# xqtr/PySpecSDR

Measured on AMD Instinct MI355X. Metric: IQ MSamples/sec end-to-end (FFT+dB+FM demod), higher is better.
Workload: dtype complex64 IQ / f64 FFT + dB + post-process + FIR + IIR / dB rows stored as f32 / int16 PCM

## Files before the change

### pyspecsdr_amd/csrc/pss_api.cpp

```cpp
#include <hip/hip_runtime.h>

#include <cstdlib>
#include <cstring>
#include <string>
#include <vector>

#include "pss_ctx.h"

static std::string g_create_err;

int pss_fail(pss_ctx *ctx, int code, const std::string &msg)
{
    if (ctx) ctx->err = msg;
    else g_create_err = msg;
    return code;
}

int pss_hip_check(pss_ctx *ctx, hipError_t e, const char *what)
{
    if (e == hipSuccess) return PSS_OK;
    return pss_fail(ctx, PSS_E_HIP, std::string(what) + ": " + hipGetErrorString(e));
}

int pss_ensure_buffer(pss_ctx *ctx, void **buf, size_t *cap, size_t bytes, const char *what)
{
    if (bytes <= *cap) return PSS_OK;
    if (*buf) {
        hipStreamSynchronize(ctx->stream);
        if (ctx->stream2) hipStreamSynchronize(ctx->stream2);
        hipFree(*buf);
        *buf = nullptr;
        *cap = 0;
    }
    hipError_t e = hipMalloc(buf, bytes);
    if (e != hipSuccess) return pss_fail(ctx, PSS_E_NOMEM, std::string(what) + " hipMalloc: " + hipGetErrorString(e));
    *cap = bytes;
    return PSS_OK;
}

int pss_ensure_scratch(pss_ctx *ctx, size_t bytes)
{
    return pss_ensure_buffer(ctx, &ctx->scratch, &ctx->scratch_bytes, bytes, "scratch");
}

void pss_time_begin(pss_ctx *ctx)
{
    if (ctx->timing && ctx->tdepth++ == 0 && ctx->tfilter.empty()) hipEventRecord(ctx->ev0, ctx->stream);
}
void pss_kernel_begin(pss_ctx *ctx, const char *name)
{
    if (!ctx->timing) return;
    ctx->kskip = !ctx->tfilter.empty() && ctx->tfilter != name;
    if (ctx->kskip) return;
    if (ctx->kused == (int)ctx->krecs.size()) {
        pss_ctx::KRec r{name, nullptr, nullptr};
        hipEventCreate(&r.e0);
        hipEventCreate(&r.e1);
        ctx->krecs.push_back(r);
    }
    ctx->krecs[ctx->kused].name = name;
    hipEventRecord(ctx->krecs[ctx->kused].e0, PSS_STREAM(ctx));
}
void pss_kernel_end(pss_ctx *ctx)
{
    if (!ctx->timing || ctx->kskip) return;
    hipEventRecord(ctx->krecs[ctx->kused].e1, PSS_STREAM(ctx));
    ctx->kused++;
}
void pss_time_end(pss_ctx *ctx)
{
    if (ctx->timing && --ctx->tdepth == 0) {
        if (ctx->tfilter.empty()) hipEventRecord(ctx->ev1, ctx->stream);
        ctx->last_ms = 0.0f;
    }
}

extern "C" int pss_device_count(void)
{
    int n = 0;
    if (hipGetDeviceCount(&n) != hipSuccess) return 0;
    return n;
}

extern "C" int pss_create(int device, pss_ctx **out)
{
    if (!out) return PSS_E_ARG;
    *out = nullptr;
    int n = 0;
    hipError_t e = hipGetDeviceCount(&n);
    if (e != hipSuccess || n <= 0)
        return pss_fail(nullptr, PSS_E_HIP, std::string("no HIP device available (libpss has no CPU fallback): ") +
                                                (e != hipSuccess ? hipGetErrorString(e) : "device count is 0"));
    if (device < 0 || device >= n) return pss_fail(nullptr, PSS_E_ARG, "device index out of range");
    int prev = -1;
    hipGetDevice(&prev);
    e = hipSetDevice(device);
    if (e != hipSuccess) return pss_fail(nullptr, PSS_E_HIP, std::string("hipSetDevice: ") + hipGetErrorString(e));
    struct Restore {
        int prev, dev;
        ~Restore() { if (prev >= 0 && prev != dev) hipSetDevice(prev); }
    } restore{prev, device};
    pss_ctx *ctx = new pss_ctx();
    ctx->device = device;
    { int cus = 0; if (hipDeviceGetAttribute(&cus, hipDeviceAttributeMultiprocessorCount, device) == hipSuccess) ctx->n_cus = cus; }
    { const char *e = getenv("PSS_NO_FUSED"); ctx->no_fused = e && e[0] == '1'; }
    e = hipStreamCreateWithFlags(&ctx->stream, hipStreamNonBlocking);
    if (e == hipSuccess) ctx->own_stream = true;
    if (e == hipSuccess) e = hipEventCreate(&ctx->ev0);
    if (e == hipSuccess) e = hipEventCreate(&ctx->ev1);
    if (e == hipSuccess) e = hipStreamCreateWithFlags(&ctx->stream2, hipStreamNonBlocking);
    if (e == hipSuccess) e = hipEventCreateWithFlags(&ctx->ev_fork, hipEventDisableTiming);
    if (e == hipSuccess) e = hipEventCreateWithFlags(&ctx->ev_join, hipEventDisableTiming);
    if (e != hipSuccess) {
        const std::string msg = std::string("context stream / event creation: ") + hipGetErrorString(e);
        if (ctx->ev0) hipEventDestroy(ctx->ev0);
        if (ctx->ev1) hipEventDestroy(ctx->ev1);
        if (ctx->ev_fork) hipEventDestroy(ctx->ev_fork);
        if (ctx->ev_join) hipEventDestroy(ctx->ev_join);
        if (ctx->stream2) hipStreamDestroy(ctx->stream2);
        if (ctx->own_stream) hipStreamDestroy(ctx->stream);
        delete ctx;
        return pss_fail(nullptr, PSS_E_HIP, msg);
    }
    *out = ctx;
    return PSS_OK;
}

extern "C" void pss_destroy(pss_ctx *ctx)
{
    if (!ctx) return;
    PssDevGuard guard(ctx->device);
    hipStreamSynchronize(ctx->stream);
    if (ctx->comm) pss_comm_free(ctx);
    for (auto &kv : ctx->tw) hipFree(kv.second);
    for (auto &kv : ctx->tw_pf) hipFree(kv.second);
    for (auto &kv : ctx->win) hipFree(kv.second);
    for (auto &kv : ctx->bs) { hipFree(kv.second.d_chirp); hipFree(kv.second.d_B); hipFree(kv.second.d_win); }
    for (auto &kv : ctx->plans) {
        hipFree(kv.second.d_leaf_off); hipFree(kv.second.d_leaf_len); hipFree(kv.second.d_node_l);
        hipFree(kv.second.d_node_r); hipFree(kv.second.d_level_start); hipFree(kv.second.d_roots);
    }
    for (auto &kv : ctx->nfm) if (kv.second.d_rev) hipFree(kv.second.d_rev);
    if (ctx->scratch) hipFree(ctx->scratch);
    if (ctx->scratch_fft) hipFree(ctx->scratch_fft);
    if (ctx->scratch_hil) hipFree(ctx->scratch_hil);
    if (ctx->scratch_iqc) hipFree(ctx->scratch_iqc);
    if (ctx->d_hann) hipFree(ctx->d_hann);
    if (ctx->d_hann_short) hipFree(ctx->d_hann_short);
    if (ctx->st_up) hipStreamDestroy(ctx->st_up);
    if (ctx->st_dn) hipStreamDestroy(ctx->st_dn);
    for (auto &e : ctx->st_ev) if (e) hipEventDestroy(e);
    for (auto &b : ctx->st_buf) if (b) hipFree(b);
    if (ctx->scratch_scan) hipFree(ctx->scratch_scan);
    if (ctx->scratch_pk) hipFree(ctx->scratch_pk);
    if (ctx->scratch_win) hipFree(ctx->scratch_win);
    if (ctx->scratch_db64) hipFree(ctx->scratch_db64);
    if (ctx->scratch_post) hipFree(ctx->scratch_post);
    if (ctx->prog) hipFree(ctx->prog);
    if (ctx->stage) hipFree(ctx->stage);
    hipEventDestroy(ctx->ev0);
    hipEventDestroy(ctx->ev1);
    hipStreamSynchronize(ctx->stream2);
    hipStreamDestroy(ctx->stream2);
    hipEventDestroy(ctx->ev_fork);
    hipEventDestroy(ctx->ev_join);
    if (ctx->ev_in) hipEventDestroy(ctx->ev_in);
    if (ctx->ev_out) hipEventDestroy(ctx->ev_out);
    for (auto &k : ctx->krecs) { hipEventDestroy(k.e0); hipEventDestroy(k.e1); }
    if (ctx->own_stream) hipStreamDestroy(ctx->stream);
    delete ctx;
}

extern "C" int pss_set_stream(pss_ctx *ctx, void *hip_stream)
{
    if (!ctx) return PSS_E_ARG;
    PSS_GUARD(ctx);
    hipStreamSynchronize(ctx->stream);
    if (ctx->own_stream) hipStreamDestroy(ctx->stream);
    ctx->stream = reinterpret_cast<hipStream_t>(hip_stream);
    ctx->own_stream = false;
    return PSS_OK;
}

extern "C" int pss_order_after(pss_ctx *ctx, void *hip_stream)
{
    if (!ctx) return PSS_E_ARG;
    PSS_GUARD(ctx);
    hipStream_t s = reinterpret_cast<hipStream_t>(hip_stream);
    if (s == ctx->stream) return PSS_OK;
    if (!ctx->ev_in) PSS_HIP(ctx, hipEventCreateWithFlags(&ctx->ev_in, hipEventDisableTiming));
    PSS_HIP(ctx, hipEventRecord(ctx->ev_in, s));
    PSS_HIP(ctx, hipStreamWaitEvent(ctx->stream, ctx->ev_in, 0));
    return PSS_OK;
}

extern "C" int pss_order_before(pss_ctx *ctx, void *hip_stream)
{
    if (!ctx) return PSS_E_ARG;
    PSS_GUARD(ctx);
    hipStream_t s = reinterpret_cast<hipStream_t>(hip_stream);
    if (s == ctx->stream) return PSS_OK;
    if (!ctx->ev_out) PSS_HIP(ctx, hipEventCreateWithFlags(&ctx->ev_out, hipEventDisableTiming));
    PSS_HIP(ctx, hipEventRecord(ctx->ev_out, ctx->stream));
    PSS_HIP(ctx, hipStreamWaitEvent(s, ctx->ev_out, 0));
    return PSS_OK;
}

extern "C" void *pss_get_stream(pss_ctx *ctx) { return ctx ? reinterpret_cast<void *>(ctx->stream) : nullptr; }

extern "C" int pss_set_option(pss_ctx *ctx, const char *key, int value)
{
    if (!ctx || !key) return PSS_E_ARG;
    if (!strcmp(key, "nfm_fused")) { ctx->no_fused = (value == 0); return PSS_OK; }
    if (!strcmp(key, "wfm_fused")) { ctx->no_wfm_fused = (value == 0); return PSS_OK; }
    if (!strcmp(key, "small_batch")) { ctx->no_small_batch = (value == 0); return PSS_OK; }
    if (!strcmp(key, "small_batch_max")) { ctx->small_batch_max = value; return PSS_OK; }
    if (!strcmp(key, "wfm_small_batch_max")) { ctx->wfm_small_batch_max = value; return PSS_OK; }
    if (!strcmp(key, "fuse_post")) { ctx->fuse_post = value != 0; return PSS_OK; }
    if (!strcmp(key, "ssb_rfft")) { ctx->ssb_rfft = value != 0; return PSS_OK; }
    if (!strcmp(key, "ssb_hilbert")) { ctx->ssb_hilbert = value != 0; return PSS_OK; }
    if (!strcmp(key, "hilbert_exact")) { ctx->hilbert_exact = value != 0; return PSS_OK; }
    if (!strcmp(key, "scan_exact")) { ctx->scan_exact = value != 0; return PSS_OK; }
    if (!strcmp(key, "db_exact")) { ctx->db_exact = value != 0; return PSS_OK; }
    if (!strcmp(key, "f64_plain")) { ctx->f64_plain = value != 0; return PSS_OK; }
    if (!strcmp(key, "wfm_corr_copy")) { ctx->wfm_corr_copy = value != 0; return PSS_OK; }
    return pss_fail(ctx, PSS_E_ARG, std::string("unknown option: ") + key);
}

extern "C" int pss_sync(pss_ctx *ctx)
{
    if (!ctx) return PSS_E_ARG;
    PSS_GUARD(ctx);
    return pss_hip_check(ctx, hipStreamSynchronize(ctx->stream), "hipStreamSynchronize");
}

extern "C" const char *pss_last_error(pss_ctx *ctx) { return ctx ? ctx->err.c_str() : g_create_err.c_str(); }

extern "C" int pss_enable_timing(pss_ctx *ctx, int on)
{
    if (!ctx) return PSS_E_ARG;
    PSS_GUARD(ctx);
    ctx->timing = on != 0;
    ctx->tdepth = 0;
    ctx->kused = 0;
    ctx->last_ms = -1.0f;
    return PSS_OK;
}

extern "C" int pss_timing_filter(pss_ctx *ctx, const char *kernel)
{
    if (!ctx) return PSS_E_ARG;
    PSS_GUARD(ctx);
    ctx->tfilter = kernel ? kernel : "";
    ctx->kused = 0;
    ctx->last_ms = -1.0f;
    return PSS_OK;
}

extern "C" float pss_last_kernel_ms(pss_ctx *ctx)
{
    if (!ctx || !ctx->timing || ctx->last_ms < 0.0f || !ctx->tfilter.empty()) return -1.0f;
    PSS_GUARD(ctx);
    if (hipEventSynchronize(ctx->ev1) != hipSuccess) return -1.0f;
    float ms = -1.0f;
    if (hipEventElapsedTime(&ms, ctx->ev0, ctx->ev1) != hipSuccess) return -1.0f;
    return ms;
}

extern "C" int pss_kernel_times(pss_ctx *ctx, char *buf, int buf_len)
{
    if (!ctx || !buf || buf_len < 1) return PSS_E_ARG;
    PSS_GUARD(ctx);
    std::string out;
    if (ctx->timing && ctx->last_ms >= 0.0f) {
        if (ctx->tfilter.empty()) hipEventSynchronize(ctx->ev1);
        else hipStreamSynchronize(ctx->stream);
        for (int i = 0; i < ctx->kused; i++) {
            float ms = 0.0f;
            if (hipEventElapsedTime(&ms, ctx->krecs[i].e0, ctx->krecs[i].e1) != hipSuccess) continue;
            out += ctx->krecs[i].name;
            out += "=" + std::to_string(ms) + ";";
        }
    }
    ctx->kused = 0;
    if ((int)out.size() + 1 > buf_len) return pss_fail(ctx, PSS_E_ARG, "buffer too small");
    memcpy(buf, out.c_str(), out.size() + 1);
    return PSS_OK;
}

namespace {
size_t up256(size_t x) { return (x + 255) & ~(size_t)255; }
}

extern "C" int pss_h_compute_fft(pss_ctx *ctx, const float *h_iq, int n, double *h_db)
{
    if (!ctx) return PSS_E_ARG;
    PSS_GUARD(ctx);
    if (!h_iq || !h_db || n < 1) return pss_fail(ctx, PSS_E_ARG, "bad arguments");
    const size_t o_db = up256(sizeof(float) * 2 * n);
    int r = pss_ensure_buffer(ctx, &ctx->stage, &ctx->stage_bytes, o_db + up256(sizeof(float) * n), "staging");
    if (r) return r;
    char *base = reinterpret_cast<char *>(ctx->stage);
    PSS_HIP(ctx, hipMemcpyAsync(base, h_iq, sizeof(float) * 2 * n, hipMemcpyHostToDevice, ctx->stream));
    r = pss_spectrum_db(ctx, reinterpret_cast<const float *>(base), 1, n, reinterpret_cast<float *>(base + o_db));
    if (r) return r;
    std::vector<float> tmp(n);
    PSS_HIP(ctx, hipMemcpyAsync(tmp.data(), base + o_db, sizeof(float) * n, hipMemcpyDeviceToHost, ctx->stream));
    PSS_HIP(ctx, hipStreamSynchronize(ctx->stream));
    for (int i = 0; i < n; i++) h_db[i] = (double)tmp[i];
    return PSS_OK;
}
// ... 521 lines not shown
```

### pyspecsdr_amd/csrc/pss_ctx.h

```cpp
#pragma once
#include <hip/hip_runtime.h>

#include <array>
#include <functional>
#include <map>
#include <string>
#include <vector>

#include "../../include/pss.h"

struct PssNfmFilt {
    double taps[65];
    double sos[24];
    double zi[8];
    double *d_rev = nullptr;
};

struct PssWfmFilt {
    double lp[18], pilot[30], lmr[30];
    double alpha;
};

struct PssPairwisePlan {
    int n_leaves = 0, n_nodes = 0, n_levels = 0, n_roots = 0;
    int wave_tree = 0;
    int *d_leaf_off = nullptr, *d_leaf_len = nullptr, *d_node_l = nullptr, *d_node_r = nullptr, *d_level_start = nullptr;
    int *d_roots = nullptr;
};

struct pss_ctx {
    int device = 0;
    hipStream_t stream = nullptr;
    bool own_stream = false;
    hipStream_t stream2 = nullptr;
    hipStream_t cur = nullptr;
    hipEvent_t ev_fork = nullptr, ev_join = nullptr;
    hipEvent_t ev_in = nullptr, ev_out = nullptr;
    int n_cus = 0;
    bool iq_c128 = false;
    int fuse_post = 1;
    double target_rate = 22050.0;
    bool wfm_correct = false;
    const float *wfm_scal = nullptr;
    bool wfm_corr_copy = false;
    float *power_out = nullptr;
    bool fork_after_fwd = false;
    bool did_fork = false;
    bool defer_bwd = false;
    std::function<int()> pending_bwd;
    std::string err;
    std::map<int, double2 *> tw;
    std::map<int, double *> win;
    std::map<int, double2 *> tw_pf;
    struct Bluestein { double2 *d_chirp; double2 *d_B; double *d_win; int M; };
    std::map<int, Bluestein> bs;
    std::map<double, PssNfmFilt> nfm;
    std::map<double, std::array<double, 65>> ssb;
    std::map<double, PssWfmFilt> wfm;
    std::map<int, PssPairwisePlan> plans;
    void *scratch = nullptr;
    size_t scratch_bytes = 0;
    void *scratch_iqc = nullptr;
    void *scratch_scan = nullptr;
    size_t scratch_scan_bytes = 0;
    void *scratch_pk = nullptr;
    size_t scratch_pk_bytes = 0;
    void *prog = nullptr;
    unsigned prog_epoch = 0;
    void *scratch_post = nullptr;
    size_t scratch_post_bytes = 0;
    void *scratch_db64 = nullptr;
    size_t scratch_db64_bytes = 0;
    void *scratch_win = nullptr;
    size_t scratch_win_bytes = 0;
    float *d_hann = nullptr;
    float hann_sum = 0.0f;
    hipStream_t st_up = nullptr, st_dn = nullptr;
    hipEvent_t st_ev[6] = {nullptr, nullptr, nullptr, nullptr, nullptr, nullptr};
    void *st_buf[18] = {};
    size_t st_cap[18] = {};
    float *d_hann_short = nullptr;
    float hann_short_sum = 0.0f;
    int hann_short_n = 0;
    size_t scratch_iqc_bytes = 0;
    void *scratch_fft = nullptr;
    size_t scratch_fft_bytes = 0;
    void *scratch_hil = nullptr;
    size_t scratch_hil_bytes = 0;
    void *stage = nullptr;
    size_t stage_bytes = 0;
    bool no_wfm_fused = false;
    long small_batch_max = 8192;
    long wfm_small_batch_max = 6000;
    bool hilbert_exact = false;
    bool ssb_rfft = true;
    bool ssb_hilbert = true;
    bool db_exact = false;
    bool f64_plain = false;
    bool scan_exact = true;
    bool no_small_batch = false;
    bool no_fused = false;
    void *comm = nullptr;
    int comm_rank = 0, comm_n = 1;
    bool timing = false;
    std::string tfilter;
    bool kskip = false;
    int tdepth = 0;
    hipEvent_t ev0 = nullptr, ev1 = nullptr;
    float last_ms = -1.0f;
    struct KRec { const char *name; hipEvent_t e0, e1; };
    std::vector<KRec> krecs;
    int kused = 0;
};

struct PssDevGuard {
    int prev = -1;
    bool switched = false;
    explicit PssDevGuard(int dev)
    {
        if (hipGetDevice(&prev) == hipSuccess && prev != dev) switched = hipSetDevice(dev) == hipSuccess;
    }
    ~PssDevGuard()
    {
        if (switched) hipSetDevice(prev);
    }
    PssDevGuard(const PssDevGuard &) = delete;
    PssDevGuard &operator=(const PssDevGuard &) = delete;
};
#define PSS_GUARD(ctx) PssDevGuard _pss_dev_guard((ctx)->device)

template <class T>
struct PssScoped {
    T &ref;
    T keep;
    PssScoped(T &r, T v) : ref(r), keep(r) { r = v; }
    ~PssScoped() { ref = keep; }
    PssScoped(const PssScoped &) = delete;
    PssScoped &operator=(const PssScoped &) = delete;
};
using PssFlagScope = PssScoped<bool>;
using PssStreamScope = PssScoped<hipStream_t>;

int pss_fail(pss_ctx *ctx, int code, const std::string &msg);
int pss_hip_check(pss_ctx *ctx, hipError_t e, const char *what);
int pss_ensure_scratch(pss_ctx *ctx, size_t bytes);
int pss_ensure_buffer(pss_ctx *ctx, void **buf, size_t *cap, size_t bytes, const char *what);
void pss_time_begin(pss_ctx *ctx);
void pss_time_end(pss_ctx *ctx);
void pss_kernel_begin(pss_ctx *ctx, const char *name);
void pss_kernel_end(pss_ctx *ctx);

#define PSS_STREAM(ctx) ((ctx)->cur ? (ctx)->cur : (ctx)->stream)

#define PSS_HIP(ctx, call)                                         \
    do {                                                           \
        int _r = pss_hip_check((ctx), (call), #call);              \
        if (_r) return _r;                                         \
    } while (0)

bool pss_hilbert_supported(int n);
int pss_hilbert_rows(pss_ctx *ctx, const double *d_x, long n_rows, int n, double *d_out, int out_mode, unsigned long long *d_maxbits,
                     int16_t *d_pcm);
int pss_fft_tables(pss_ctx *ctx, int n, const double2 **tw, const double **win);
bool pss_post_sel_serves(int n_fft, bool f64);
bool pss_spec_post_serves(const pss_ctx *ctx, int n_fft);
int pss_spec_post_chain(pss_ctx *ctx, const float *d_iq, long n_frames, int n_fft, float *d_db32, double *d_db64, double *d_lo, double *d_hi, int n_halo,
                        int window, int display, int disp_h, int disp_w, int8_t *d_a, int8_t *d_b, double *d_vals);
int pss_chain_vals_f32(pss_ctx *ctx, const float *d_db, long n_frames, int n_fft, float *d_lo, float *d_hi, int n_halo, int window, int display,
                       int disp_h, int disp_w, int8_t *d_a, int8_t *d_b, double *d_vals);
int pss_chain_vals_f64(pss_ctx *ctx, const double *d_db, long n_frames, int n_fft, double *d_lo, double *d_hi, int n_halo, int window, int display,
                       int disp_h, int disp_w, int8_t *d_a, int8_t *d_b, double *d_vals);
bool pss_ssb_fused_supported(int n);
double pss_np_tan(double x);
double pss_np_exp(double x);
int pss_ssb_hilbert_fused(pss_ctx *ctx, const float *d_iq, long n_rows, int n, const double *taps65, double *d_audio, int16_t *d_pcm);
```

### pyspecsdr_amd/csrc/pss_fft.hip

```cpp
#include <hip/hip_runtime.h>

#include <cmath>
#include <vector>

#include "pss_ctx.h"
#include "pss_fft_r16.h"
#include "pss_fft_xl.h"
#include "pss_post.h"
#include "pss_spec_post.h"
#include "pss_hilbert.h"
#include "pss_hilbert_pf.h"

namespace {

constexpr int TPB = 256;

inline int spec_flags(const pss_ctx *ctx) { return (ctx->scan_exact ? pss_r16::FLAG_SCAN_EXACT : 0) | (ctx->db_exact ? pss_r16::FLAG_DB_EXACT : 0); }
constexpr int LOG_NSUB_MAX = 12;
constexpr int STAGE_MAX_N = 16384;
constexpr int PT = 1024;

__device__ __forceinline__ double2 cmul(double2 a, double2 b)
{
    return make_double2(a.x * b.x - a.y * b.y, a.x * b.y + a.y * b.x);
// ... 1491 lines not shown
        pss_time_end(ctx);
        return pss_hip_check(ctx, hipGetLastError(), "k_disp_vals_win launch");
    }
    int r = pss_ensure_buffer(ctx, &ctx->scratch_win, &ctx->scratch_win_bytes, (size_t)n_frames * 2 * sizeof(double), "window extremes");
    if (r) { pss_time_end(ctx); return r; }
    double *wlo = reinterpret_cast<double *>(ctx->scratch_win), *whi = wlo + n_frames;
    pss_kernel_begin(ctx, "k_slide_extremes");
    hipLaunchKernelGGL(pss_post::k_slide_extremes<T>, dim3((unsigned)((n_frames + 255) / 256 < 4096 ? (n_frames + 255) / 256 : 4096)),
                       dim3(256), 0, PSS_STREAM(ctx), d_lo, d_hi, n_frames, n_halo, window, wlo, whi);
    pss_kernel_end(ctx);
    const long cells = n_frames * disp_w;
    pss_kernel_begin(ctx, "k_disp_rows");
    const dim3 dgrid((unsigned)((cells + 255) / 256 < 16384 ? (cells + 255) / 256 : 16384));
    if (d_thr)
        hipLaunchKernelGGL((pss_post::k_disp_rows<T, MODE, true>), dgrid, dim3(256), 0, PSS_STREAM(ctx), d_post, wlo, whi, n_frames, len,
                           disp_w, disp_h, d_a, d_b, d_thr);
    else
        hipLaunchKernelGGL((pss_post::k_disp_rows<T, MODE>), dgrid, dim3(256), 0, PSS_STREAM(ctx), d_post, wlo, whi, n_frames, len, disp_w,
                           disp_h, d_a, d_b, (const T *)nullptr);
    pss_kernel_end(ctx);
    pss_time_end(ctx);
    return pss_hip_check(ctx, hipGetLastError(), "k_disp_rows launch");
}

}

extern "C" int pss_spectrum_db_post(pss_ctx *ctx, const float *d_iq, long n_frames, int n_fft, float *d_db, float *d_post,
                                    float *d_row_lo, float *d_row_hi)
{
    if (!ctx) return PSS_E_ARG;
    PSS_GUARD(ctx);
    if (n_frames < 0 || (n_frames > 0 && (!d_iq || !d_db || !d_post))) return pss_fail(ctx, PSS_E_ARG, "pss_spectrum_db_post: null buffer");
    if ((d_row_lo == nullptr) != (d_row_hi == nullptr)) return pss_fail(ctx, PSS_E_ARG, "row extremes: pass both arrays or neither");
    if (n_frames == 0) return PSS_OK;
    int r = pss_spectrum_db(ctx, d_iq, n_frames, n_fft, d_db);
    if (!r) r = spectrum_post(ctx, d_db, n_frames, n_fft, d_post, d_row_lo, d_row_hi);
    return r;
}

extern "C" int pss_spectrum_post(pss_ctx *ctx, const float *d_db, long n_frames, int n_fft, float *d_post)
{
    if (!ctx) return PSS_E_ARG;
    PSS_GUARD(ctx);
    return spectrum_post(ctx, d_db, n_frames, n_fft, d_post, nullptr, nullptr);
}

extern "C" int pss_spectrum_post_extremes(pss_ctx *ctx, const float *d_db, long n_frames, int n_fft, float *d_post, float *d_row_lo,
                                          float *d_row_hi)
{
    if (!ctx) return PSS_E_ARG;
    PSS_GUARD(ctx);
    if (n_frames > 0 && (!d_row_lo || !d_row_hi)) return pss_fail(ctx, PSS_E_ARG, "null row-extremes array");
    return spectrum_post(ctx, d_db, n_frames, n_fft, d_post, d_row_lo, d_row_hi);
}

extern "C" int pss_row_extremes(pss_ctx *ctx, const float *d_rows, long n_rows, int len, float *d_row_lo, float *d_row_hi)
{
    if (!ctx) return PSS_E_ARG;
    PSS_GUARD(ctx);
    return row_extremes<float>(ctx, d_rows, n_rows, len, d_row_lo, d_row_hi);
}
extern "C" int pss_row_extremes_f64(pss_ctx *ctx, const double *d_rows, long n_rows, int len, double *d_row_lo, double *d_row_hi)
{
    if (!ctx) return PSS_E_ARG;
    PSS_GUARD(ctx);
    return row_extremes<double>(ctx, d_rows, n_rows, len, d_row_lo, d_row_hi);
}

extern "C" int pss_spectrum_post_f64(pss_ctx *ctx, const double *d_db, long n_frames, int n_fft, double *d_post, double *d_row_lo, double *d_row_hi)
{
    if (!ctx) return PSS_E_ARG;
    PSS_GUARD(ctx);
    if (n_frames < 0 || n_fft < 5 || (n_frames > 0 && (!d_db || !d_post))) return pss_fail(ctx, PSS_E_ARG, "pss_spectrum_post_f64: bad argument");
    if ((d_row_lo == nullptr) != (d_row_hi == nullptr)) return pss_fail(ctx, PSS_E_ARG, "pss_spectrum_post_f64: row_lo and row_hi go together");
    if (n_frames == 0) return PSS_OK;
    if (!ctx->f64_plain && n_fft >= 8 && post_sel_serves(n_fft, true)) {
        pss_time_begin(ctx);
        const int rq = post_sel_any<double>(ctx, d_db, n_frames, n_fft, d_post, d_row_lo, d_row_hi, nullptr, nullptr, 0);
        pss_time_end(ctx);
        return rq;
    }
    pss_time_begin(ctx);
    pss_kernel_begin(ctx, "k_post_f64");
    hipLaunchKernelGGL(k_post_f64, dim3((unsigned)(n_frames < 2048 ? n_frames : 2048)), dim3(256), 0, PSS_STREAM(ctx), d_db, d_post, n_fft, n_frames);
    pss_kernel_end(ctx);
    int r = pss_hip_check(ctx, hipGetLastError(), "k_post_f64 launch");
    if (!r && d_row_lo) r = row_extremes<double>(ctx, d_post, n_frames, n_fft - 4, d_row_lo, d_row_hi);
    pss_time_end(ctx);
    return r;
}

extern "C" int pss_spectrum_post_thresholds(pss_ctx *ctx, const float *d_db, long n_frames, int n_fft, float *d_row_thr, float *d_row_lo,
                                            float *d_row_hi)
{
    if (!ctx) return PSS_E_ARG;
    PSS_GUARD(ctx);
    if (n_frames > 0 && (!d_row_thr || !d_row_lo || !d_row_hi)) return pss_fail(ctx, PSS_E_ARG, "pss_spectrum_post_thresholds: null buffer");
    return spectrum_post(ctx, d_db, n_frames, n_fft, nullptr, d_row_lo, d_row_hi, d_row_thr);
}
extern "C" int pss_waterfall_rows_db(pss_ctx *ctx, const float *d_db, long n_frames, int n_fft, const float *d_row_thr, const float *d_row_lo,
                                     const float *d_row_hi, int n_halo, int window, int disp_w, int8_t *d_glyph, int8_t *d_colour)
{
    if (!ctx) return PSS_E_ARG;
    PSS_GUARD(ctx);
    if (n_frames > 0 && !d_row_thr) return pss_fail(ctx, PSS_E_ARG, "pss_waterfall_rows_db: null thresholds");
    return display_rows<float, 0>(ctx, d_db, n_frames, n_fft - 4, d_row_lo, d_row_hi, n_halo, window, 1, disp_w, d_glyph, d_colour, d_row_thr);
}
extern "C" int pss_persistence_rows_db(pss_ctx *ctx, const float *d_db, long n_frames, int n_fft, const float *d_row_thr,
                                       const float *d_row_lo, const float *d_row_hi, int n_halo, int window, int disp_h, int disp_w, int8_t *d_y)
{
    if (!ctx) return PSS_E_ARG;
    PSS_GUARD(ctx);
    if (n_frames > 0 && !d_row_thr) return pss_fail(ctx, PSS_E_ARG, "pss_persistence_rows_db: null thresholds");
    return display_rows<float, 1>(ctx, d_db, n_frames, n_fft - 4, d_row_lo, d_row_hi, n_halo, window, disp_h, disp_w, d_y, nullptr, d_row_thr);
}

bool pss_post_sel_serves(int n_fft, bool f64) { return n_fft >= 8 && post_sel_serves(n_fft, f64); }
template <class TR>
static int chain_vals(pss_ctx *ctx, const TR *d_db, long n_frames, int n_fft, TR *d_lo, TR *d_hi, int n_halo, int window, int display, int disp_h,
                      int disp_w, int8_t *d_a, int8_t *d_b, double *d_vals)
{
    if (n_frames == 0) return PSS_OK;
    pss_time_begin(ctx);
    int r = post_sel_any<TR>(ctx, d_db, n_frames, n_fft, (TR *)nullptr, d_lo + n_halo, d_hi + n_halo, (TR *)nullptr, d_vals, disp_w);
    if (!r) r = display ? display_rows<TR, 1>(ctx, (const TR *)nullptr, n_frames, n_fft - 4, d_lo, d_hi, n_halo, window, disp_h, disp_w, d_a, nullptr, (const TR *)nullptr, d_vals)
                        : display_rows<TR, 0>(ctx, (const TR *)nullptr, n_frames, n_fft - 4, d_lo, d_hi, n_halo, window, 1, disp_w, d_a, d_b, (const TR *)nullptr, d_vals);
    pss_time_end(ctx);
    return r;
}
int pss_chain_vals_f32(pss_ctx *ctx, const float *d_db, long n_frames, int n_fft, float *d_lo, float *d_hi, int n_halo, int window, int display,
                       int disp_h, int disp_w, int8_t *d_a, int8_t *d_b, double *d_vals)
{
    return chain_vals<float>(ctx, d_db, n_frames, n_fft, d_lo, d_hi, n_halo, window, display, disp_h, disp_w, d_a, d_b, d_vals);
}
int pss_chain_vals_f64(pss_ctx *ctx, const double *d_db, long n_frames, int n_fft, double *d_lo, double *d_hi, int n_halo, int window, int display,
                       int disp_h, int disp_w, int8_t *d_a, int8_t *d_b, double *d_vals)
{
    return chain_vals<double>(ctx, d_db, n_frames, n_fft, d_lo, d_hi, n_halo, window, display, disp_h, disp_w, d_a, d_b, d_vals);
}

bool pss_spec_post_serves(const pss_ctx *ctx, int n_fft) { return n_fft == 1024 && !ctx->f64_plain; }
int pss_spec_post_chain(pss_ctx *ctx, const float *d_iq, long n_frames, int n_fft, float *d_db32, double *d_db64, double *d_lo, double *d_hi,
                        int n_halo, int window, int display, int disp_h, int disp_w, int8_t *d_a, int8_t *d_b, double *d_vals)
{
    if (!pss_spec_post_serves(ctx, n_fft) || (!d_db32 && !d_db64)) return pss_fail(ctx, PSS_E_ARG, "fused transform + post-process: 1024-point frames, a row buffer");
    if (n_frames == 0) return PSS_OK;
    const double2 *tw;
    const double *win;
    int r = pss_fft_tables(ctx, n_fft, &tw, &win);
    if (r) return r;
    using C = pss_r16::Cfg<2>;
    auto kern = d_db32 ? (d_db64 ? pss_sp::k_spectrum_post<true, true> : pss_sp::k_spectrum_post<true, false>) : pss_sp::k_spectrum_post<false, true>;
    const size_t lds = (size_t)C::FPW * C::EX * sizeof(double2) + (size_t)C::TW2 * sizeof(double2);
    const long cap = 256L * 2 * 2;
    if (lds > 64 * 1024) PSS_HIP(ctx, hipFuncSetAttribute(reinterpret_cast<const void *>(kern), hipFuncAttributeMaxDynamicSharedMemorySize, (int)lds));
    const long groups = (n_frames + C::FPW - 1) / C::FPW;
    pss_time_begin(ctx);
    pss_kernel_begin(ctx, "k_spectrum_post");
    hipLaunchKernelGGL(kern, dim3((unsigned)(groups < cap ? groups : cap)), dim3(256), lds, PSS_STREAM(ctx), reinterpret_cast<const float2 *>(d_iq), d_db32,
                       d_db64, tw, win, n_frames, d_lo + n_halo, d_hi + n_halo, d_vals, disp_w);
    pss_kernel_end(ctx);
    r = pss_hip_check(ctx, hipGetLastError(), "k_spectrum_post launch");
    if (!r) r = display ? display_rows<double, 1>(ctx, (const double *)nullptr, n_frames, n_fft - 4, d_lo, d_hi, n_halo, window, disp_h, disp_w, d_a, nullptr, (const double *)nullptr, d_vals)
                        : display_rows<double, 0>(ctx, (const double *)nullptr, n_frames, n_fft - 4, d_lo, d_hi, n_halo, window, 1, disp_w, d_a, d_b, (const double *)nullptr, d_vals);
    pss_time_end(ctx);
    return r;
}

extern "C" int pss_waterfall_rows(pss_ctx *ctx, const float *d_post, long n_frames, int len, const float *d_row_lo,
                                  const float *d_row_hi, int n_halo, int window, int disp_w, int8_t *d_glyph, int8_t *d_colour)
{
    if (!ctx) return PSS_E_ARG;
    PSS_GUARD(ctx);
    return display_rows<float, 0>(ctx, d_post, n_frames, len, d_row_lo, d_row_hi, n_halo, window, 1, disp_w, d_glyph, d_colour);
}
extern "C" int pss_waterfall_rows_f64(pss_ctx *ctx, const double *d_post, long n_frames, int len, const double *d_row_lo,
                                      const double *d_row_hi, int n_halo, int window, int disp_w, int8_t *d_glyph, int8_t *d_colour)
{
    if (!ctx) return PSS_E_ARG;
    PSS_GUARD(ctx);
    return display_rows<double, 0>(ctx, d_post, n_frames, len, d_row_lo, d_row_hi, n_halo, window, 1, disp_w, d_glyph, d_colour);
}
extern "C" int pss_persistence_rows(pss_ctx *ctx, const float *d_post, long n_frames, int len, const float *d_row_lo,
                                    const float *d_row_hi, int n_halo, int window, int disp_h, int disp_w, int8_t *d_y)
{
    if (!ctx) return PSS_E_ARG;
    PSS_GUARD(ctx);
    return display_rows<float, 1>(ctx, d_post, n_frames, len, d_row_lo, d_row_hi, n_halo, window, disp_h, disp_w, d_y, nullptr);
}
extern "C" int pss_persistence_rows_f64(pss_ctx *ctx, const double *d_post, long n_frames, int len, const double *d_row_lo,
                                        const double *d_row_hi, int n_halo, int window, int disp_h, int disp_w, int8_t *d_y)
{
    if (!ctx) return PSS_E_ARG;
    PSS_GUARD(ctx);
    return display_rows<double, 1>(ctx, d_post, n_frames, len, d_row_lo, d_row_hi, n_halo, window, disp_h, disp_w, d_y, nullptr);
}

extern "C" int pss_waterfall_cells(pss_ctx *ctx, const float *d_rows, int n_rows, int len, int disp_h, int disp_w,
                                   int8_t *d_glyph, int8_t *d_colour)
{
    if (!ctx) return PSS_E_ARG;
    PSS_GUARD(ctx);
    if (!d_rows || !d_glyph || !d_colour || n_rows < 1 || len < 2 || disp_h < 1 || disp_w < 1)
        return pss_fail(ctx, PSS_E_ARG, "bad waterfall arguments");
    pss_kernel_begin(ctx, "k_cells");
    hipLaunchKernelGGL((k_cells<float, 0>), dim3(1), dim3(1024), 0, PSS_STREAM(ctx), d_rows, n_rows, len, disp_h, disp_w,
                       d_glyph, d_colour, 0, n_rows);
    pss_kernel_end(ctx);
    return pss_hip_check(ctx, hipGetLastError(), "k_cells launch");
}

extern "C" int pss_persistence_cells(pss_ctx *ctx, const float *d_rows, int n_rows, int len, int disp_h, int disp_w,
                                     int8_t *d_colour)
{
    if (!ctx) return PSS_E_ARG;
    PSS_GUARD(ctx);
    if (!d_rows || !d_colour || n_rows < 1 || len < 2 || disp_h < 1 || disp_w < 1)
        return pss_fail(ctx, PSS_E_ARG, "bad persistence arguments");
    pss_kernel_begin(ctx, "k_cells");
    hipLaunchKernelGGL((k_cells<float, 1>), dim3(1), dim3(1024), 0, PSS_STREAM(ctx), d_rows, n_rows, len, disp_h, disp_w,
                       (int8_t *)nullptr, d_colour, 0, n_rows);
    pss_kernel_end(ctx);
    return pss_hip_check(ctx, hipGetLastError(), "k_cells launch");
}

template <class T>
static int launch_spectrogram(pss_ctx *ctx, const T *d_rows, long n_rows, int len, int disp_h, int disp_w, int8_t *d_glyph,
                              int8_t *d_colour, double *d_range)
{
    if (!ctx) return PSS_E_ARG;
    PSS_GUARD(ctx);
    if (!d_rows || !d_glyph || !d_colour || n_rows < 0 || len < 2 || disp_h < 1 || disp_w < 1)
        return pss_fail(ctx, PSS_E_ARG, "bad spectrogram arguments");
    if (n_rows == 0) return PSS_OK;
    pss_kernel_begin(ctx, "k_spectrogram");
    hipLaunchKernelGGL(k_spectrogram<T>, dim3((unsigned)(n_rows < 4096 ? n_rows : 4096)), dim3(len <= 4096 ? 256 : 1024), 0,
                       PSS_STREAM(ctx), d_rows, n_rows, len, disp_h, disp_w, d_glyph, d_colour, d_range);
    pss_kernel_end(ctx);
    return pss_hip_check(ctx, hipGetLastError(), "k_spectrogram launch");
}

extern "C" int pss_spectrogram_cells(pss_ctx *ctx, const float *d_rows, long n_rows, int len, int disp_h, int disp_w,
                                     int8_t *d_glyph, int8_t *d_colour, double *d_range)
{
    return launch_spectrogram<float>(ctx, d_rows, n_rows, len, disp_h, disp_w, d_glyph, d_colour, d_range);
}

extern "C" int pss_spectrogram_cells_f64(pss_ctx *ctx, const double *d_rows, long n_rows, int len, int disp_h, int disp_w,
                                         int8_t *d_glyph, int8_t *d_colour, double *d_range)
{
    return launch_spectrogram<double>(ctx, d_rows, n_rows, len, disp_h, disp_w, d_glyph, d_colour, d_range);
}

__global__ __launch_bounds__(256) void k_vector(const float2 *__restrict__ iq, int n, int max_h, int max_w, int8_t *__restrict__ grid)
{
    const int cx = max_w / 2, cy = max_h / 2, scale = (max_w < max_h ? max_w : max_h) / 4;
    for (int k = blockIdx.x * blockDim.x + threadIdx.x; k < n; k += gridDim.x * blockDim.x) {
        const float2 v = iq[k];
        const float fx = __fadd_rn((float)cx, __fmul_rn(v.x, (float)scale)), fy = __fsub_rn((float)cy, __fmul_rn(v.y, (float)scale));
        if (!isfinite(fx) || !isfinite(fy)) continue;
        const int x = (int)fx, y = (int)fy;
        if (x >= 0 && x < max_w && y >= 0 && y < max_h) grid[y * max_w + x] = 1;
    }
}

extern "C" int pss_vector_cells(pss_ctx *ctx, const float *d_iq, int n, int max_h, int max_w, int8_t *d_grid)
{
    if (!ctx) return PSS_E_ARG;
    PSS_GUARD(ctx);
    if (!d_iq || !d_grid || n < 0 || max_h < 1 || max_w < 1) return pss_fail(ctx, PSS_E_ARG, "bad vector-display arguments");
    PSS_HIP(ctx, hipMemsetAsync(d_grid, 0, (size_t)max_h * max_w, PSS_STREAM(ctx)));
    if (n == 0) return PSS_OK;
    pss_kernel_begin(ctx, "k_vector");
    hipLaunchKernelGGL(k_vector, dim3((unsigned)((n + 255) / 256 < 1024 ? (n + 255) / 256 : 1024)), dim3(256), 0, PSS_STREAM(ctx),
                       reinterpret_cast<const float2 *>(d_iq), n, max_h, max_w, d_grid);
    pss_kernel_end(ctx);
    return pss_hip_check(ctx, hipGetLastError(), "k_vector launch");
}

template <class T>
static int launch_gradient(pss_ctx *ctx, const T *d_rows, int n_rows, int len, int disp_h, int disp_w, int8_t *d_glyph,
                           int8_t *d_colour)
{
    if (!ctx) return PSS_E_ARG;
    PSS_GUARD(ctx);
    if (!d_rows || !d_glyph || !d_colour || n_rows < 1 || len < 2 || disp_h < 1 || disp_w < 1)
        return pss_fail(ctx, PSS_E_ARG, "bad waterfall arguments");
    pss_kernel_begin(ctx, "k_cells");
    hipLaunchKernelGGL((k_cells<T, 2>), dim3(1), dim3(1024), 0, PSS_STREAM(ctx), d_rows, n_rows, len, disp_h, disp_w, d_glyph,
                       d_colour, 0, n_rows);
    pss_kernel_end(ctx);
    return pss_hip_check(ctx, hipGetLastError(), "k_cells launch");
}
extern "C" int pss_gradient_cells(pss_ctx *ctx, const float *d_rows, int n_rows, int len, int disp_h, int disp_w,
                                  int8_t *d_glyph, int8_t *d_colour)
{
    return launch_gradient<float>(ctx, d_rows, n_rows, len, disp_h, disp_w, d_glyph, d_colour);
}
extern "C" int pss_gradient_cells_f64(pss_ctx *ctx, const double *d_rows, int n_rows, int len, int disp_h, int disp_w,
                                      int8_t *d_glyph, int8_t *d_colour)
{
    return launch_gradient<double>(ctx, d_rows, n_rows, len, disp_h, disp_w, d_glyph, d_colour);
}

template <class T>
static int launch_surface(pss_ctx *ctx, const T *d_row, int len, int max_h, int max_w, int8_t *d_colour)
{
    if (!ctx) return PSS_E_ARG;
    PSS_GUARD(ctx);
    if (!d_row || !d_colour || len < 2 || max_h < 4 || max_w < 10) return pss_fail(ctx, PSS_E_ARG, "bad surface arguments");
    int r = pss_ensure_buffer(ctx, &ctx->scratch_fft, &ctx->scratch_fft_bytes, (size_t)max_h * max_w * sizeof(int), "surface keys");
    if (r) return r;
    pss_kernel_begin(ctx, "k_cells");
    hipLaunchKernelGGL((k_cells<T, 3>), dim3(1), dim3(1024), 0, PSS_STREAM(ctx), d_row, 1, len, max_h, max_w,
                       reinterpret_cast<int8_t *>(ctx->scratch_fft), d_colour, 0, 1);
// ... 99 lines not shown
```

### pyspecsdr_amd/csrc/pss_spec_post.h

```cpp
#pragma once

namespace pss_sp {

using namespace pss_r16;

template <bool ROW32, bool ROW64>
__global__ __launch_bounds__(256, 2) void k_spectrum_post(const float2 *__restrict__ iq, float *__restrict__ db32, double *__restrict__ db64,
                                                       const double2 *__restrict__ tw, const double *__restrict__ win, long n_frames,
                                                       double *__restrict__ row_lo, double *__restrict__ row_hi, double *__restrict__ vals,
                                                       int disp_w)
{
    using C = Cfg<2>;
    constexpr int R3 = C::R3, T = C::T, N = C::N, FPW = C::FPW;
    static_assert(T == 64, "a frame is one wavefront");
    constexpr int EPL = 16;
    using PC = pss_post::PostCfg<EPL, double>;
    static_assert((size_t)(T + 1) * PC::S * sizeof(double) <= (size_t)C::EX * sizeof(double2), "the staged row fits the frame's exchange buffer");
    extern __shared__ __align__(16) unsigned char smem[];
    double2 *ex_all = reinterpret_cast<double2 *>(smem);
    double2 *tw2 = ex_all + (size_t)FPW * C::EX;
    const int tid = threadIdx.x;
    const int fl = __builtin_amdgcn_readfirstlane(tid / T);
    const int t = tid % T;
    double2 *ex = ex_all + (size_t)fl * C::EX;
    double *stage = reinterpret_cast<double *>(ex);
    double2 tw1[16];
    double w[16];
    tw1[0] = make_double2(1.0, 0.0);
#pragma unroll
    for (int k2 = 1; k2 < 16; k2++) tw1[k2] = tw[(size_t)t * k2];
#pragma unroll
    for (int n2 = 0; n2 < 16; n2++) w[n2] = win[t + T * n2];
    if (tid < R3 * 16) {
        const int m1 = tid / 16, j2 = tid % 16;
        tw2[C::tw2_slot(tid)] = tw[(size_t)(m1 * j2) * 16];
    }
    __syncthreads();
    const long groups = (n_frames + FPW - 1) / FPW;
    float2 nx[16];
    auto fetch = [&](long g) {
        const long f = g * FPW + fl;
        const float2 *x = iq + (size_t)(f < n_frames ? f : 0) * N;
#pragma unroll
        for (int n2 = 0; n2 < 16; n2++) nx[n2] = x[t + T * n2];
    };
    if ((long)blockIdx.x < groups) fetch(blockIdx.x);
    int phase = 0;
    for (long g = blockIdx.x; g < groups; g += gridDim.x) {
        const long f = g * FPW + fl;
        const bool valid = f < n_frames;
        double2 v[16];
#pragma unroll
        for (int n2 = 0; n2 < 16; n2++) v[n2] = make_double2((double)nx[n2].x * w[n2], (double)nx[n2].y * w[n2]);
        if (g + gridDim.x < groups) fetch(g + gridDim.x);
        const long f_first = g * FPW;
        const long rows_here = n_frames - f_first < FPW ? n_frames - f_first : FPW;
        const __amdgpu_buffer_rsrc_t ro32 = make_rsrc((ROW32 && db32) ? db32 + (size_t)f_first * N : nullptr, (ROW32 && db32) ? (unsigned)(rows_here * N * 4) : 0u);
        const __amdgpu_buffer_rsrc_t ro64 = make_rsrc((ROW64 && db64) ? db64 + (size_t)f_first * N : nullptr, (ROW64 && db64) ? (unsigned)(rows_here * N * 8) : 0u);
        const int lane_el = fl * N + t;
        double dbv[16];
        auto emit = [&](int i, int k, double2 X) {
            const double d64 = db64_of_exact(power_of(X));
            const int e0 = ((k - t) + N / 2) & (N - 1);
            if constexpr (ROW64) buf_store_f64(ro64, lane_el * 8, e0 * 8, d64);
            if constexpr (ROW32) buf_store_f32(ro32, lane_el * 4, e0 * 4, (float)d64);
            dbv[i] = d64;
        };
        r16_core<2, true>(v, ex, tw1, tw2, t, emit);
        frame_sync<true>();
#pragma unroll
        for (int i = 0; i < 16; i++) {
            const int c = i / R3, j1 = i % R3;
            const int e = (((256 * j1 + T * c) + N / 2) & (N - 1)) + t;
            stage[(e / EPL) * PC::S + (e % EPL)] = dbv[i];
        }
        frame_sync<true>();
        if (valid) {
            int slot[PC::Q];
#pragma unroll
            for (int j = 0; j < PC::Q; j++) slot[j] = 0;
            pss_post::post_row_staged<EPL, 1, true, double>(stage, slot, t, N - 4, nullptr, fl, t, phase, nullptr, row_lo, row_hi, f, nullptr, vals, disp_w);
        }
        frame_sync<true>();
    }
}

}
```

Measured before the change: 70090.

## Replace static grid-stride frame loop with per-wavefront atomic ticket work stealing

The fused spectrum+dB+post kernel now has each wavefront draw its next frame from per-head atomic counters instead of walking a fixed grid-stride sequence. Frames are split into 8 contiguous shares, and counters persist across launches through host-tracked base offsets. The grid cap is tied to the CU count rather than a hard constant. This aims to balance load and remove tail imbalance between CUs, at the cost of an atomic per frame and extra host bookkeeping that assumes every launch completes its draws.

```diff
diff --git a/pyspecsdr_amd/csrc/pss_api.cpp b/pyspecsdr_amd/csrc/pss_api.cpp
--- a/pyspecsdr_amd/csrc/pss_api.cpp
+++ b/pyspecsdr_amd/csrc/pss_api.cpp
@@ -157,6 +157,7 @@
     if (ctx->scratch_db64) hipFree(ctx->scratch_db64);
     if (ctx->scratch_post) hipFree(ctx->scratch_post);
     if (ctx->prog) hipFree(ctx->prog);
+    for (auto &kv : ctx->tickets) hipFree(kv.second.d);
     if (ctx->stage) hipFree(ctx->stage);
     hipEventDestroy(ctx->ev0);
     hipEventDestroy(ctx->ev1);
diff --git a/pyspecsdr_amd/csrc/pss_ctx.h b/pyspecsdr_amd/csrc/pss_ctx.h
--- a/pyspecsdr_amd/csrc/pss_ctx.h
+++ b/pyspecsdr_amd/csrc/pss_ctx.h
@@ -67,6 +67,8 @@
     size_t scratch_pk_bytes = 0;
     void *prog = nullptr;
     unsigned prog_epoch = 0;
+    struct Tickets { unsigned *d = nullptr; unsigned next[8] = {}; };
+    std::map<hipStream_t, Tickets> tickets;
     void *scratch_post = nullptr;
     size_t scratch_post_bytes = 0;
     void *scratch_db64 = nullptr;
diff --git a/pyspecsdr_amd/csrc/pss_fft.hip b/pyspecsdr_amd/csrc/pss_fft.hip
--- a/pyspecsdr_amd/csrc/pss_fft.hip
+++ b/pyspecsdr_amd/csrc/pss_fft.hip
@@ -1667,15 +1667,32 @@
     using C = pss_r16::Cfg<2>;
     auto kern = d_db32 ? (d_db64 ? pss_sp::k_spectrum_post<true, true> : pss_sp::k_spectrum_post<true, false>) : pss_sp::k_spectrum_post<false, true>;
     const size_t lds = (size_t)C::FPW * C::EX * sizeof(double2) + (size_t)C::TW2 * sizeof(double2);
-    const long cap = 256L * 2 * 2;
     if (lds > 64 * 1024) PSS_HIP(ctx, hipFuncSetAttribute(reinterpret_cast<const void *>(kern), hipFuncAttributeMaxDynamicSharedMemorySize, (int)lds));
     const long groups = (n_frames + C::FPW - 1) / C::FPW;
+    const long cap = 2L * (ctx->n_cus > 0 ? ctx->n_cus : 256);
+    const int grid = (int)(groups < cap ? groups : cap);
+    const int heads = grid < pss_sp::TICKET_HEADS ? grid : pss_sp::TICKET_HEADS;
+    hipStream_t st = PSS_STREAM(ctx);
+    pss_ctx::Tickets &tk = ctx->tickets[st];
+    if (!tk.d) {
+        PSS_HIP(ctx, hipMalloc(&tk.d, sizeof(unsigned) * pss_sp::TICKET_STRIDE * pss_sp::TICKET_HEADS));
+        PSS_HIP(ctx, hipMemsetAsync(tk.d, 0, sizeof(unsigned) * pss_sp::TICKET_STRIDE * pss_sp::TICKET_HEADS, st));
+        for (unsigned &v : tk.next) v = 0;
+    }
+    pss_sp::TicketBase base;
+    for (int h = 0; h < pss_sp::TICKET_HEADS; h++) base.v[h] = tk.next[h];
     pss_time_begin(ctx);
     pss_kernel_begin(ctx, "k_spectrum_post");
-    hipLaunchKernelGGL(kern, dim3((unsigned)(groups < cap ? groups : cap)), dim3(256), lds, PSS_STREAM(ctx), reinterpret_cast<const float2 *>(d_iq), d_db32,
-                       d_db64, tw, win, n_frames, d_lo + n_halo, d_hi + n_halo, d_vals, disp_w);
+    hipLaunchKernelGGL(kern, dim3((unsigned)grid), dim3(256), lds, st, reinterpret_cast<const float2 *>(d_iq), d_db32, d_db64, tw, win, n_frames,
+                       d_lo + n_halo, d_hi + n_halo, d_vals, disp_w, tk.d, base, heads);
     pss_kernel_end(ctx);
     r = pss_hip_check(ctx, hipGetLastError(), "k_spectrum_post launch");
+    if (!r) {
+        for (int h = 0; h < heads; h++) {
+            const pss_sp::TicketShare sh = pss_sp::ticket_share(n_frames, grid, heads, h, C::FPW);
+            tk.next[h] += (unsigned)(sh.frames > sh.waves ? sh.frames : sh.waves);
+        }
+    }
     if (!r) r = display ? display_rows<double, 1>(ctx, (const double *)nullptr, n_frames, n_fft - 4, d_lo, d_hi, n_halo, window, disp_h, disp_w, d_a, nullptr, (const double *)nullptr, d_vals)
                         : display_rows<double, 0>(ctx, (const double *)nullptr, n_frames, n_fft - 4, d_lo, d_hi, n_halo, window, 1, disp_w, d_a, d_b, (const double *)nullptr, d_vals);
     pss_time_end(ctx);
diff --git a/pyspecsdr_amd/csrc/pss_spec_post.h b/pyspecsdr_amd/csrc/pss_spec_post.h
--- a/pyspecsdr_amd/csrc/pss_spec_post.h
+++ b/pyspecsdr_amd/csrc/pss_spec_post.h
@@ -4,11 +4,24 @@
 
 using namespace pss_r16;
 
+constexpr int TICKET_HEADS = 8;
+constexpr int TICKET_STRIDE = 32;
+struct TicketBase { unsigned v[TICKET_HEADS]; };
+struct TicketShare { int first, frames, waves; };
+__host__ __device__ inline TicketShare ticket_share(long n_frames, int grid, int heads, int h, int fpw)
+{
+    TicketShare s;
+    s.first = (int)(n_frames * h / heads);
+    s.frames = (int)(n_frames * (h + 1) / heads) - s.first;
+    s.waves = (grid - h + heads - 1) / heads * fpw;
+    return s;
+}
+
 template <bool ROW32, bool ROW64>
 __global__ __launch_bounds__(256, 2) void k_spectrum_post(const float2 *__restrict__ iq, float *__restrict__ db32, double *__restrict__ db64,
                                                        const double2 *__restrict__ tw, const double *__restrict__ win, long n_frames,
                                                        double *__restrict__ row_lo, double *__restrict__ row_hi, double *__restrict__ vals,
-                                                       int disp_w)
+                                                       int disp_w, unsigned *__restrict__ tickets, TicketBase base, int heads)
 {
     using C = Cfg<2>;
     constexpr int R3 = C::R3, T = C::T, N = C::N, FPW = C::FPW;
@@ -36,38 +49,47 @@
         tw2[C::tw2_slot(tid)] = tw[(size_t)(m1 * j2) * 16];
     }
     __syncthreads();
-    const long groups = (n_frames + FPW - 1) / FPW;
+    const int h = (int)(blockIdx.x % (unsigned)heads);
+    const TicketShare share = ticket_share(n_frames, (int)gridDim.x, heads, h, FPW);
+    unsigned *const counter = tickets + h * TICKET_STRIDE;
+    const unsigned b = base.v[h];
     float2 nx[16];
-    auto fetch = [&](long g) {
-        const long f = g * FPW + fl;
-        const float2 *x = iq + (size_t)(f < n_frames ? f : 0) * N;
+    auto fetch = [&](int f) {
+        const float2 *x = iq + (size_t)f * N;
 #pragma unroll
         for (int n2 = 0; n2 < 16; n2++) nx[n2] = x[t + T * n2];
     };
-    if ((long)blockIdx.x < groups) fetch(blockIdx.x);
+    auto draw = [&]() -> unsigned {
+        unsigned c = 0;
+        if (t == 0) c = __builtin_amdgcn_atomic_inc32(counter, 0xffffffffu, __ATOMIC_RELAXED, "agent");
+        return c;
+    };
+    auto position = [&](unsigned c) { return share.waves + (int)((unsigned)__builtin_amdgcn_readfirstlane((int)c) - b); };
+    int pos = (int)(blockIdx.x / (unsigned)heads) * FPW + fl;
+    if (pos < share.frames) fetch(share.first + pos);
+    int pos_next = position(draw());
     int phase = 0;
-    for (long g = blockIdx.x; g < groups; g += gridDim.x) {
-        const long f = g * FPW + fl;
-        const bool valid = f < n_frames;
+    while (pos < share.frames) {
+        const int f = share.first + pos;
         double2 v[16];
 #pragma unroll
         for (int n2 = 0; n2 < 16; n2++) v[n2] = make_double2((double)nx[n2].x * w[n2], (double)nx[n2].y * w[n2]);
-        if (g + gridDim.x < groups) fetch(g + gridDim.x);
-        const long f_first = g * FPW;
-        const long rows_here = n_frames - f_first < FPW ? n_frames - f_first : FPW;
-        const __amdgpu_buffer_rsrc_t ro32 = make_rsrc((ROW32 && db32) ? db32 + (size_t)f_first * N : nullptr, (ROW32 && db32) ? (unsigned)(rows_here * N * 4) : 0u);
-        const __amdgpu_buffer_rsrc_t ro64 = make_rsrc((ROW64 && db64) ? db64 + (size_t)f_first * N : nullptr, (ROW64 && db64) ? (unsigned)(rows_here * N * 8) : 0u);
-        const int lane_el = fl * N + t;
+        const bool more = pos_next < share.frames;
+        if (more) fetch(share.first + pos_next);
+        const __amdgpu_buffer_rsrc_t ro32 = make_rsrc((ROW32 && db32) ? db32 + (size_t)f * N : nullptr, (ROW32 && db32) ? (unsigned)(N * 4) : 0u);
+        const __amdgpu_buffer_rsrc_t ro64 = make_rsrc((ROW64 && db64) ? db64 + (size_t)f * N : nullptr, (ROW64 && db64) ? (unsigned)(N * 8) : 0u);
         double dbv[16];
         auto emit = [&](int i, int k, double2 X) {
             const double d64 = db64_of_exact(power_of(X));
             const int e0 = ((k - t) + N / 2) & (N - 1);
-            if constexpr (ROW64) buf_store_f64(ro64, lane_el * 8, e0 * 8, d64);
-            if constexpr (ROW32) buf_store_f32(ro32, lane_el * 4, e0 * 4, (float)d64);
+            if constexpr (ROW64) buf_store_f64(ro64, t * 8, e0 * 8, d64);
+            if constexpr (ROW32) buf_store_f32(ro32, t * 4, e0 * 4, (float)d64);
             dbv[i] = d64;
         };
         r16_core<2, true>(v, ex, tw1, tw2, t, emit);
         frame_sync<true>();
+        unsigned drawn = 0;
+        if (more) drawn = draw();
 #pragma unroll
         for (int i = 0; i < 16; i++) {
             const int c = i / R3, j1 = i % R3;
@@ -75,13 +97,15 @@
             stage[(e / EPL) * PC::S + (e % EPL)] = dbv[i];
         }
         frame_sync<true>();
-        if (valid) {
+        {
             int slot[PC::Q];
 #pragma unroll
             for (int j = 0; j < PC::Q; j++) slot[j] = 0;
             pss_post::post_row_staged<EPL, 1, true, double>(stage, slot, t, N - 4, nullptr, fl, t, phase, nullptr, row_lo, row_hi, f, nullptr, vals, disp_w);
         }
         frame_sync<true>();
+        pos = pos_next;
+        if (more) pos_next = position(drawn);
     }
 }
 
```

Result: no change. 70510, median of 6 (+0.6%).
